# buwantaiji/FermiFlow

Hardware: AMD Instinct MI355X
Metric: walker-steps/sec (full VMC iteration: 100 MCMC steps + generate + E_loc + grad + Adam) (higher is better)
Workload: dtype f64

## Files before the change

### fermiflow_amd/csrc/ff_cnf_fwd.hip

```cpp
#include <atomic>
#include "ff_common.h"
#include "ff_ode.h"
#include "ff_slater.h"
#include "ff_eloc_ws.h"
#define FF_RADIAL_BUILD_KERNELS
#include "ff_radial.h"

#ifdef FF_STAMPS
#define FF_STAMP(i) do { unsigned long long t_ = __builtin_amdgcn_s_memtime(); stamp_acc[i] += t_ - stamp_prev; stamp_prev = t_; } while (0)
#else
#define FF_STAMP(i) do { } while (0)
#endif

#ifndef FF_TAB_MODE
#define FF_TAB_MODE(MODE) true
#endif

#include "ff_fwd_args.h"

#ifndef FF_FORM_EARLY
#define FF_FORM_EARLY 1
#endif
#ifndef FF_SWEEP_CH
#define FF_SWEEP_CH 2
#endif
#ifndef FF_FWD_WAVES_PER_SIMD
#define FF_FWD_WAVES_PER_SIMD 1
#endif
#ifndef FF_FLOW_WAVES
#define FF_FLOW_WAVES 3
#endif
#ifndef FF_FWD_STATIC
#define FF_FWD_STATIC(N, D, MODE, TAB) ((MODE) == 0 && (TAB) && (N) * (D) <= 12)
#endif
template <int N, int D, int MODE_, bool TAB>
__global__ void __launch_bounds__(FF_WAVE, ((MODE_ == 0 || MODE_ == FF_MODE_FRAMES) && TAB && N * D <= 12) ? FF_FLOW_WAVES : FF_FWD_WAVES_PER_SIMD)
ff_ode_fwd_kernel(ff_fwd_args A) {
  constexpr bool FRAMES = MODE_ == FF_MODE_FRAMES;
  constexpr int MODE = FRAMES ? 0 : MODE_;
  if constexpr (MODE == 0) FF_SETPRIO();
  using Gm = ff_geom<N, D>;
  constexpr int M = Gm::M, G = Gm::G, P = Gm::P, R = Gm::RA;
  constexpr int NH = MODE == 0 ? 1 : (MODE == 1 ? 2 : 4);
  constexpr int NV = MODE == 0 ? 1 : (MODE == 1 ? 2 : M + 5);
  constexpr int IDL = MODE == 1 ? 1 : M + 3;

  __shared__ ff_wtab s_w[TAB ? 1 : 2][TAB ? 1 : FF_HPAD];
  __shared__ double s_e2[TAB ? 1 : 64];
  __shared__ double s_z[G][M], s_kb[G][M], s_err[G][M];
  constexpr bool JET = (MODE == 2);
  constexpr bool LEAN = (MODE == 0 && TAB);
  __shared__ __attribute__((aligned(16))) double s_rr[(JET || LEAN) ? 1 : G][(JET || LEAN) ? 1 : R][2];
  __shared__ __attribute__((aligned(16))) double s_hd[JET ? 1 : G][JET ? 1 : R][NH];
  constexpr int RECW = (D + 7 + 1) & ~1;
  constexpr int RECS0 = R * RECW, RECS = RECS0 + ((RECS0 % 4 == 2) ? 0 : ((RECS0 % 4 == 0) ? 2 : 1));
  static_assert(!JET || ((2 * RECS) % 32) % 8 == 4, "record stride");
  __shared__ __attribute__((aligned(16))) double s_rec[JET ? G * RECS : 1];
  constexpr int QTW = ((3 * N > M) ? 3 * N + 1 : M + 1) | 1;
  constexpr int TROW = N * 3 * D + 1;
  static_assert(N * TROW <= M * QTW, "T must fit the transposition buffer");
  __shared__ __attribute__((aligned(16))) double s_qt[JET ? G * M * QTW : 1];
  __shared__ double s_zero[LEAN ? (D > 2 ? D : 2) : 1];
  __shared__ int s_pa[R], s_pb[R], s_any;
  __shared__ double s_rmin[G][R];
  static_assert(MODE != 2 || M <= 12, "the column-sweep local-energy kernel serves at most 12 coordinates");
  constexpr bool LDS_STATE = (MODE == 2);
  __shared__ double s_yv[LDS_STATE ? NV : 1][FF_WAVE], s_cv[LDS_STATE ? NV : 1][FF_WAVE];

  const int lane = threadIdx.x;
  const int g = lane / M, i = lane % M;
  const bool ingrp = g < G;
  const int gg = ingrp ? g : 0;
  const int ai = i / D, ci = i % D;
  const double* __restrict__ rtab = A.net.radial_table;
  if constexpr (TAB) {
    if (rtab[3] != 0.0) {
      if (lane == 0 && blockIdx.x == 0) *A.evt = A.evt_id;
      return;
    }
  } else {
    if (A.evt && *A.evt != A.evt_id) return;
    ff_fill_exp2_table(s_e2, lane);
    ff_load_weights(s_w, A.net, lane);
  }
  bool off_table = false;
  if constexpr (LEAN) { if (lane < (D > 2 ? D : 2)) s_zero[lane] = 0.0; }
  if (lane == 0) {
    int p = 0;
    for (int a = 0; a < N; a++)
      for (int b = a + 1; b < N; b++) { s_pa[p] = a; s_pb[p] = b; p++; }
    for (int a = 0; a < N; a++) { if (P + a < R) { s_pa[P + a] = a; s_pb[P + a] = -1; } }
  }
  FF_WG1_SYNC();
  const int He = A.net.He, Hm = A.net.Hm;
  const bool has_mu = Hm > 0;
  const int nrad = has_mu ? (P + N) : P;
  const double tab_inv_h = TAB ? rtab[0] : 0.0, tab_h = TAB ? rtab[1] : 0.0;
  auto heads = [&](int t, double r, double* hd) {
    if constexpr (TAB) {
      if (!ff_heads_table<NH>(rtab, tab_inv_h, tab_h, t, r, hd)) {
        off_table = true;
#pragma unroll
        for (int m = 0; m < NH; m++) hd[m] = 0.0;
      }
    } else {
      ff_heads<NH, FF_TAB_MODE(MODE)>(s_w[t], s_e2, t ? Hm : He, r, hd);
    }
  };
  const double rtol = A.rtol, atol = A.atol;
  constexpr double NT = MODE == 0 ? M : (MODE == 1 ? M + 1 : M * (M + 4) + 1);
  const int64_t ngroups = (A.B + G - 1) / G;
  __shared__ int s_st[4];
  if (lane < 4) s_st[lane] = 0;
  constexpr int NQ = (G * R + FF_WAVE - 1) / FF_WAVE;
  int rq_id[NQ];
#pragma unroll
  for (int qk = 0; qk < NQ; qk++) {
    const int q = lane + qk * FF_WAVE;
    const bool act = q < G * nrad;
    const int qg = act ? q / nrad : 0, p = act ? q - qg * nrad : 0;
    rq_id[qk] = act ? (qg | (s_pa[p] << 4) | ((s_pb[p] < 0 ? 15 : s_pb[p]) << 8) | (p << 12)) : -1;
  }
#ifdef FF_STAMPS
  unsigned long long stamp_acc[9] = {0, 0, 0, 0, 0, 0, 0, 0, 0}, stamp_prev = __builtin_amdgcn_s_memtime();
  unsigned long long stage_acc[9] = {0, 0, 0, 0, 0, 0, 0, 0, 0}, stage_cnt[9] = {0, 0, 0, 0, 0, 0, 0, 0, 0};
  const unsigned long long stamp_t0 = stamp_prev, stamp_r0 = __builtin_readcyclecounter() * 0 + wall_clock64();
#endif

  __shared__ long long s_next;
  for (int64_t grp = blockIdx.x;; grp += gridDim.x) {
    if (A.queue) {
      FF_WG1_SYNC();
      if (lane == 0) s_next = (long long)atomicAdd(A.queue + (TAB ? 0 : 1), 1ULL);
      FF_WG1_SYNC();
      grp = s_next;
    }
    if (grp >= ngroups) break;
    const int64_t bq = grp * G + g;
    const bool inb = ingrp && bq < A.B;
    const int64_t b = ff_opt_load(A.order, inb, bq, A.y_in, (int32_t)bq);
    const bool valid = inb && !(MODE == 2 && N <= 3 && A.heavy_mode == 2 && ff_opt_load(A.wclass, inb, b, A.y_in, (int32_t)0) >= A.heavy_class);
    ff_lane_vec<NV, LDS_STATE> y(&s_yv[0][0], lane), c3(&s_cv[0][0], lane);
    double c0[NV], c1[NV], c2[NV];
#pragma unroll
    for (int v = 0; v < NV; v++) { y[v] = 0.0; c0[v] = 0.0; c1[v] = 0.0; c2[v] = 0.0; c3[v] = 0.0; }
    y[0] = ff_opt_load(A.y_in, valid, b * M + i, A.y_in, 0.25 * (i + 1) + 0.125 * ((i * 7) % 5));
    if constexpr (MODE == 2) {
#pragma unroll
      for (int k = 0; k < M; k++) y[1 + k] = (k == i) ? 1.0 : 0.0;
    }
    std::conditional_t<FRAMES, ff_frame_stepper, ff_stepper> S;
    if constexpr (FRAMES) {
      S.begin(A.ta, A.tb, valid, A.nframes);
      if (valid) A.y_out[b * M + i] = y[0];
    } else {
      S.begin(A.ta, A.tb, valid);
    }
    const bool loose = MODE == 2 && ff_opt_load(A.wclass, valid, b, A.y_in, (int32_t)0x7fffffff) <= A.sens_class;
    const double hwarm = ff_open_step(ff_opt_load(A.h_init, valid, A.h_scale < 0.0 ? 0 : b, A.y_in, 0.0) * (loose ? A.h_scale_loose : fabs(A.h_scale)),
                                      A.ta, A.tb, MODE == 2 ? 0 : A.h_equal);
    const bool warm = hwarm > 0.0;
    double hmax_acc = 0.0;
    int s = -2, nev = 0;
    double h0v = 0.0, d1v = 0.0;
    double rmin_q[NQ];
#pragma unroll
    for (int k = 0; k < NQ; k++) rmin_q[k] = 1e300;

    auto group_sum = [&](double part) -> double {
      if (ingrp) s_err[g][i] = part;
      FF_WG1_SYNC();
      double t = 0.0;
#pragma unroll
      for (int j = 0; j < M; j++) t += s_err[gg][j];
      FF_WG1_SYNC();
      return t;
    };
    const double sens_w = loose ? A.sens_w : 1.0;
    auto wgt = [&](int v) -> double {
      if (MODE >= 1 && v == IDL && i != 0) return 0.0;
      return (MODE == 2 && v >= 1) ? sens_w : 1.0;
    };

    constexpr bool STATIC_STAGES = FF_FWD_STATIC(N, D, MODE, TAB);
    auto evaluate = [&](auto stage_tag) -> bool {
      constexpr int SG = decltype(stage_tag)::value;
      if constexpr (SG == FF_STAGE_DYN && STATIC_STAGES) FF_ASSUME(s <= 0);
      const int sv = SG == FF_STAGE_DYN ? s : SG;
      const double h = S.h;
      double gy = 1.0, g0 = 0.0, g1 = 0.0, g2 = 0.0;
      switch (sv) {
        case -1: g0 = h0v * S.dir; break;
        case 1: g0 = h * FF_A10; break;
        case 2: g0 = h * FF_A20; g1 = h * FF_A21; break;
        case 3: g0 = h * FF_A30; g1 = h * FF_A31; g2 = h * FF_A32; break;
        case 4: gy = 0.0; g0 = 1.0; break;
        case 5: gy = 0.0; g1 = 1.0; break;
        case 6: gy = 0.0; g2 = 1.0; break;
        default: break;
      }
      auto form = [&](double* dst, const int v0, const int v1, const int stride) {
#pragma unroll
        for (int v = v0; v < v1; v += stride) dst[v] = fma(g2, c2[v], fma(g1, c1[v], fma(g0, c0[v], gy * y[v])));
      };
      FF_STAMP(0);
      FF_WG1_SYNC();
      {
        double pub[NV];
        form(pub, 0, MODE == 2 ? M + 2 : 1, MODE == 2 ? M + 1 : 1);
        if (ingrp) {
          s_z[g][i] = pub[0];
          if constexpr (MODE == 2) s_kb[g][i] = pub[M + 1];
        }
      }
      FF_WG1_SYNC();
      FF_STAMP(1);
      double rq_rho[NQ][D], rq_dk[JET ? NQ : 1][D], rq_r[NQ], rq_ri[NQ], rq_T[NQ][TAB ? NH + 5 : 1], rq_dr[NQ];
      bool rq_ok[NQ];
#pragma unroll
      for (int qk = 0; qk < NQ; qk++) {
        const int id = rq_id[qk];
        const bool act = id >= 0;
        const int qg = act ? (id & 15) : 0, a = act ? ((id >> 4) & 15) : 0, bq = act ? ((id >> 8) & 15) : 15;
        const bool pair = bq != 15;
        const int bb = pair ? bq : a;
        double r2 = 0.0;
        const double* zpart = pair ? &s_z[qg][bb * D] : s_zero;
#pragma unroll
        for (int c = 0; c < D; c++) {
          if constexpr (LEAN) rq_rho[qk][c] = s_z[qg][a * D + c] - zpart[c];
          else rq_rho[qk][c] = s_z[qg][a * D + c] - (pair ? s_z[qg][bb * D + c] : 0.0);
          if constexpr (JET) rq_dk[qk][c] = s_kb[qg][a * D + c] - (pair ? s_kb[qg][bb * D + c] : 0.0);
          r2 = fma(rq_rho[qk][c], rq_rho[qk][c], r2);
        }
        ff_sqrt_rcp(r2, rq_r[qk], rq_ri[qk]);
        if (act) rmin_q[qk] = fmin(rmin_q[qk], rq_r[qk]);
        rq_dr[qk] = 0.0;
        rq_ok[qk] = true;
        if constexpr (TAB) {
          if constexpr (LEAN) {
            rq_ok[qk] = ff_table_fetch_always<NH>(rtab, tab_inv_h, tab_h, pair ? 0 : 1, rq_r[qk], rq_T[qk], rq_dr[qk]);
            off_table |= act & !rq_ok[qk];
          } else {
            rq_ok[qk] = ff_table_fetch<NH>(rtab, tab_inv_h, tab_h, pair ? 0 : 1, rq_r[qk], rq_T[qk], rq_dr[qk]);
            if (act && !rq_ok[qk]) off_table = true;
          }
        }
      }
      double in[NV], out[NV];
      if constexpr (MODE == 2 && FF_FORM_EARLY) form(in, 0, NV, 1);
#pragma unroll
      for (int qk = 0; qk < NQ; qk++) {
        const int id = rq_id[qk];
        if (id < 0) break;
        const int qg = id & 15, a = (id >> 4) & 15, bq = (id >> 8) & 15, p = id >> 12;
        const bool pair = bq != 15;
        const int bb = pair ? bq : a;
        const double* rho = rq_rho[qk];
        const double r = rq_r[qk], ri = rq_ri[qk];
        double hd[NH];
        if constexpr (LEAN) {
          ff_table_eval<NH>(rq_T[qk], rq_dr[qk], hd);
#pragma unroll
          for (int m = 0; m < NH; m++) hd[m] = rq_ok[qk] ? hd[m] : 0.0;
        } else if constexpr (TAB) {
          if (rq_ok[qk]) ff_table_eval<NH>(rq_T[qk], rq_dr[qk], hd);
          else {
#pragma unroll
            for (int m = 0; m < NH; m++) hd[m] = 0.0;
          }
        } else {
          heads(pair ? 0 : 1, r, hd);
        }
        if constexpr (!JET) {
          if constexpr (!LEAN) {
            s_rr[qg][p][0] = r;
            s_rr[qg][p][1] = ri;
          }
#pragma unroll
          for (int m = 0; m < NH; m++) s_hd[qg][p][m] = hd[m];
        } else {
          const double cf = pair ? 2.0 : 1.0;
          const double f0 = hd[0], f1 = hd[1], f2 = hd[NH > 2 ? 2 : 0], f3 = hd[NH > 3 ? 3 : 0];
          const double Ac = cf * fma(f2, r, (1.0 + D) * f1), Bc = cf * fma(f3, r, (2.0 + D) * f2);
          double* rec = &s_rec[qg * RECS + p * RECW];
#pragma unroll
          for (int c = 0; c < D; c++) rec[c] = rho[c];
          rec[D] = ri; rec[D + 1] = f0; rec[D + 2] = f1; rec[D + 3] = f2; rec[D + 4] = Ac; rec[D + 5] = Bc;
          rec[D + 6] = cf * fma(f1, r, D * f0);
          const double* dk = rq_dk[qk];
          double rdk = 0.0;
#pragma unroll
          for (int c = 0; c < D; c++) rdk = fma(rho[c], dk[c], rdk);
          const double F1k = f1 * (rdk * ri), gq = Ac * ri;
          double* Ta = &s_qt[qg * M * QTW + a * TROW + bb * 3 * D];
          double* Tb = &s_qt[qg * M * QTW + bb * TROW + a * 3 * D];
#pragma unroll
          for (int c = 0; c < D; c++) {
            const double pv = f0 * rho[c], pw = fma(F1k, rho[c], f0 * dk[c]), pg = gq * rho[c];
            Ta[c] = pv; Ta[D + c] = pw; Ta[2 * D + c] = pg;
            if (pair) { Tb[c] = -pv; Tb[D + c] = -pw; Tb[2 * D + c] = -pg; }
          }
        }
      }
      FF_WG1_SYNC();
      nev++;
      FF_STAMP(2);
      if constexpr (!(MODE == 2 && FF_FORM_EARLY)) form(in, 0, NV, 1);
      FF_STAMP(6);
      const double* sz = s_z[gg];
      double sumq = 0.0, ddiv = 0.0, qdiv = 0.0, divv = 0.0;
      double vi = 0.0, dvk = 0.0, gdi = 0.0;
      if constexpr (MODE == 2) {
        {
          const double* T = &s_qt[gg * M * QTW + ai * TROW + ci];
#pragma unroll
          for (int j = 0; j < N; j++) {
            const bool use = has_mu || j != ai;
            const double tv = T[j * 3 * D], tw = T[j * 3 * D + D], tg = T[j * 3 * D + 2 * D];
            vi += use ? tv : 0.0; dvk += use ? tw : 0.0; gdi += use ? tg : 0.0;
          }
        }
        FF_WG1_SYNC();
        double du[M], qv[M];
#pragma unroll
        for (int k = 0; k < M; k++) { du[k] = 0.0; qv[k] = 0.0; }
        const double* u = &in[1];
        constexpr int CH = FF_SWEEP_CH, RT = P + N, NCH = (RT + CH - 1) / CH;
        constexpr ff_pair_table<N> PT{};
        double hb[2][CH][RECW];
        auto load_chunk = [&](int c, double (*buf)[RECW]) {
#pragma unroll
          for (int q = 0; q < CH; q++) {
            const int p = c * CH + q;
            if (p < RT) {
#pragma unroll
              for (int m = 0; m < D + 7; m++) buf[q][m] = s_rec[gg * RECS + p * RECW + m];
            }
          }
        };
        load_chunk(0, hb[0]);
#pragma unroll
        for (int c = 0; c < NCH; c++) {
          if (c + 1 < NCH) load_chunk(c + 1, hb[(c + 1) & 1]);
#pragma unroll
          for (int q = 0; q < CH; q++) {
            const int p = c * CH + q;
            if (p < RT && (p < P || has_mu)) {
              const bool pair = p < P;
              const int a = pair ? PT.a[p < P ? p : 0] : p - P, bq = pair ? PT.b[p < P ? p : 0] : 0;
              const double* hq = hb[c & 1][q];
              const double* rho = hq;
              const double ri = hq[D], f0 = hq[D + 1], f1 = hq[D + 2], f2 = hq[D + 3], Ac = hq[D + 4], Bc = hq[D + 5];
              double dl[D], rd = 0.0, dd = 0.0;
#pragma unroll
              for (int cc = 0; cc < D; cc++) {
                dl[cc] = pair ? u[a * D + cc] - u[bq * D + cc] : u[a * D + cc];
                rd = fma(rho[cc], dl[cc], rd);
                dd = fma(dl[cc], dl[cc], dd);
              }
              const double r1 = rd * ri, r1s = r1 * r1;
              const double r2q = (dd - r1s) * ri;
              const double F1 = f1 * r1, F2 = fma(f2, r1s, f1 * r2q), F1x2 = F1 + F1;
#pragma unroll
              for (int cc = 0; cc < D; cc++) {
                const double g1 = fma(F1, rho[cc], f0 * dl[cc]);
                const double g2 = fma(F2, rho[cc], F1x2 * dl[cc]);
                du[a * D + cc] += g1;
                qv[a * D + cc] += g2;
                if (pair) { du[bq * D + cc] -= g1; qv[bq * D + cc] -= g2; }
              }
              ddiv = fma(Ac, r1, ddiv);
              qdiv = fma(Bc, r1s, fma(Ac, r2q, qdiv));
              divv += hq[D + 6];
            }
          }
          FF_SCHED_FENCE();
        }
        FF_STAMP(7);
#pragma unroll
        for (int k = 0; k < M; k++) out[1 + k] = du[k];
        if (ingrp) {
#pragma unroll
          for (int k = 0; k < M; k++) s_qt[(g * M + i) * QTW + k] = qv[k];
        }
        FF_WG1_SYNC();
#pragma unroll
        for (int j = 0; j < M; j++) sumq += s_qt[(gg * M + j) * QTW + i];
        FF_STAMP(3);
      } else {
        if constexpr (MODE == 1) {
          for (int p = 0; p < nrad; p++) {
            const double c = p < P ? 2.0 : 1.0;
            divv = fma(c, fma(s_hd[gg][p][NH > 1 ? 1 : 0], s_rr[gg][p][0], D * s_hd[gg][p][0]), divv);
          }
        }
        const double zc = sz[ai * D + ci];
#pragma unroll
        for (int bq = 0; bq < N; bq++) {
          const bool self = (bq == ai);
          const int lo = bq < ai ? bq : ai, hi = bq < ai ? ai : bq;
          const int p = self ? 0 : ff_pair_index(N, lo, hi);
          if constexpr (LEAN) {
            const double* hp = self ? s_zero : &s_hd[gg][p][0];
            vi = fma(*hp, zc - sz[bq * D + ci], vi);
          } else {
            vi = fma(self ? 0.0 : s_hd[gg][p][0], zc - sz[bq * D + ci], vi);
          }
        }
        if (has_mu) vi = fma(s_hd[gg][P + ai][0], zc, vi);
      }
      out[0] = vi;
      if constexpr (MODE == 1) out[1] = -divv;
      if constexpr (MODE == 2) {
        out[M + 1] = sumq + dvk;
        out[M + 2] = -ddiv;
        out[M + 3] = -divv;
        out[M + 4] = -fma(gdi, in[M + 1], qdiv);
      }
      FF_STAMP(4);
#if defined(FF_STAMPS) && defined(FF_STAMPS_TRACE)
      const int s_prev = sv;
#endif
      if (sv == -2) {
#pragma unroll
        for (int v = 0; v < NV; v++) c0[v] = out[v];
        double p0 = 0.0, p1 = 0.0;
#pragma unroll
        for (int v = 0; v < NV; v++) {
          const double isc = wgt(v) * ff_rcp(fma(fabs(y[v]), rtol, atol));
          p0 = fma(y[v] * isc, y[v] * isc, p0);
          p1 = fma(c0[v] * isc, c0[v] * isc, p1);
        }
        const double d0 = sqrt(group_sum(p0) * (1.0 / NT));
        d1v = sqrt(group_sum(p1) * (1.0 / NT));
        h0v = S.h0(d0, d1v);
        s = -1;
        if (!ff_wave_or(&s_any, lane, (!S.done && !warm) ? 1 : 0)) {
          S.habs = fmin(hwarm, S.interval);
          S.plan();
          s = 1;
        }
      } else if (sv == -1) {
        double p2 = 0.0;
#pragma unroll
        for (int v = 0; v < NV; v++) {
          const double t = (out[v] - c0[v]) * wgt(v) * ff_rcp(fma(fabs(y[v]), rtol, atol));
          p2 = fma(t, t, p2);
        }
        const double d2 = sqrt(group_sum(p2) * (1.0 / NT)) / h0v;
        S.init_habs(h0v, d1v, d2);
        if (warm) S.habs = fmin(hwarm, S.interval);
        S.plan();
        s = 1;
      } else if (sv == 0) {
#pragma unroll
        for (int v = 0; v < NV; v++) c0[v] = out[v];
        s = 1;
      } else if (sv == 1) {
#pragma unroll
        for (int v = 0; v < NV; v++) c1[v] = out[v];
        s = 2;
      } else if (sv == 2) {
#pragma unroll
        for (int v = 0; v < NV; v++) c2[v] = out[v];
        s = 3;
      } else if (sv == 3) {
#pragma unroll
        for (int v = 0; v < NV; v++) {
          const double k0v = c0[v], k1v = c1[v], k2v = c2[v], k3v = out[v];
          c0[v] = fma(h, FF_A40 * k0v + FF_A41 * k1v + FF_A42 * k2v + FF_A43 * k3v, y[v]);
          c1[v] = fma(h, FF_A50 * k0v + FF_A51 * k1v + FF_A52 * k2v + FF_A53 * k3v, y[v]);
          c2[v] = fma(h, FF_B0 * k0v + FF_B2 * k2v + FF_B3 * k3v, y[v]);
          c3[v] = h * (FF_E0 * k0v + FF_E2 * k2v + FF_E3 * k3v);
          if constexpr (STATIC_STAGES) { FF_OPAQUE(c0[v]); FF_OPAQUE(c1[v]); FF_OPAQUE(c2[v]); }
        }
        s = 4;
      } else if (sv == 4) {
#pragma unroll
        for (int v = 0; v < NV; v++) {
          c1[v] = fma(h * FF_A54, out[v], c1[v]);
          c2[v] = fma(h * FF_B4, out[v], c2[v]);
          c3[v] = fma(h * FF_E4, out[v], c3[v]);
          if constexpr (STATIC_STAGES) { FF_OPAQUE(c1[v]); FF_OPAQUE(c2[v]); }
        }
        s = 5;
      } else if (sv == 5) {
#pragma unroll
        for (int v = 0; v < NV; v++) {
          c2[v] = fma(h * FF_B5, out[v], c2[v]);
          c3[v] = fma(h * FF_E5, out[v], c3[v]);
          if constexpr (STATIC_STAGES) { FF_OPAQUE(c2[v]); }
        }
        s = 6;
      } else {
        double pe = 0.0;
#pragma unroll
        for (int v = 0; v < NV; v++) {
          const double e = fma(h * FF_E6, out[v], c3[v]);
          const double t = e * wgt(v) * ff_rcp(fma(fmax(fabs(y[v]), fabs(in[v])), rtol, atol));
          pe = fma(t, t, pe);
        }
        const double err = sqrt(group_sum(pe) * (1.0 / NT));
        const bool was_active = !S.done;
        const bool acc = S.decide(err, A.max_steps);
        if (acc) hmax_acc = fmax(hmax_acc, fabs(h));
        if (acc) {
#pragma unroll
          for (int v = 0; v < NV; v++) { y[v] = in[v]; c0[v] = out[v]; }
        }
        if constexpr (FRAMES) {
          if (valid && S.landed >= 0) A.y_out[((int64_t)S.landed * A.B + b) * M + i] = y[0];
        }
        S.plan();
        const int any = ff_wave_or(&s_any, lane, S.done ? 0 : ((was_active && !acc) ? 3 : 1));
        s = (any & 2) ? 0 : 1;
        if (!any) { FF_STAMP(5); return true; }
      }
#if defined(FF_STAMPS) && defined(FF_STAMPS_TRACE)
      { unsigned long long t_ = __builtin_amdgcn_s_memtime(); stage_acc[s_prev + 2] += t_ - stamp_prev; stage_cnt[s_prev + 2]++; }
#endif
      FF_STAMP(5);
      return false;
    };
    if constexpr (STATIC_STAGES) {
#pragma unroll 1
      for (;;) {
#pragma unroll 1
        while (s <= 0) evaluate(ff_stage_c<FF_STAGE_DYN>{});
        evaluate(ff_stage_c<1>{});
        evaluate(ff_stage_c<2>{});
        evaluate(ff_stage_c<3>{});
        evaluate(ff_stage_c<4>{});
        evaluate(ff_stage_c<5>{});
        if (evaluate(ff_stage_c<6>{})) break;
      }
    } else {
#pragma unroll 1
      for (;;) {
        if (evaluate(ff_stage_c<FF_STAGE_DYN>{})) break;
      }
    }
    if (A.wcost) {
#pragma unroll
      for (int qk = 0; qk < NQ; qk++) {
        if (rq_id[qk] >= 0) s_rmin[rq_id[qk] & 15][rq_id[qk] >> 12] = rmin_q[qk];
      }
      FF_WG1_SYNC();
    }
    if (valid) {
      const bool failed = S.fail != 0;
#ifdef FF_NO_POISON
      const double bad = 0.0;
#else
      const double bad = failed ? __builtin_nan("") : 0.0;
#endif
      if constexpr (FRAMES) {
        for (int k = S.kf; k < A.nframes; k++) A.y_out[((int64_t)k * A.B + b) * M + i] = y[0] + bad;
      } else {
        A.y_out[b * M + i] = y[0] + bad;
      }
      if constexpr (MODE >= 1) { if (i == 0) A.dl_out[b] = y[IDL] + bad; }
      if constexpr (MODE == 2) {
#pragma unroll
        for (int k = 0; k < M; k++) A.Jt[(b * M + i) * M + k] = y[1 + k];
        A.kbar[b * M + i] = y[M + 1];
        A.dD[b * M + i] = y[M + 2];
        A.Lpart[b * M + i] = y[M + 4];
      }
      if (i == 0) {
        if (A.h_out) A.h_out[b] = hmax_acc > 0.0 ? hmax_acc : hwarm;
        if (A.wcost) {
          double rm = 1e300;
          for (int p = 0; p < nrad; p++) rm = fmin(rm, s_rmin[g][p]);
          A.wcost[b] = ff_cost_class(S.nacc + S.nrej, rm);
        }
        if (A.stats) { atomicAdd(&s_st[0], nev); atomicMax(&s_st[1], S.nacc); atomicAdd(&s_st[2], S.nrej); if (failed) atomicMax(&s_st[3], 1); }
      }
    }
    FF_WG1_SYNC();
  }
#ifdef FF_STAMPS
  if (A.stats && lane == 0)
    for (int q = 0; q < 9; q++) atomicAdd((unsigned long long*)(A.stats + 8) + q, stamp_acc[q]);
  if (A.stats && lane == 0 && blockIdx.x == 0) {
    A.stats[26] = (int)(__builtin_amdgcn_s_memtime() - stamp_t0);
    A.stats[27] = (int)(wall_clock64() - stamp_r0);
  }
#ifdef FF_STAMPS_TRACE
  if (A.stats && lane == 0)
    for (int q = 0; q < 9; q++) {
      atomicAdd((unsigned long long*)(A.stats + 65600) + q, stage_acc[q]);
      atomicAdd((unsigned long long*)(A.stats + 65600) + 9 + q, stage_cnt[q]);
    }
#endif
#ifdef FF_STAMPS_TRACE
  if (A.stats && lane == 0 && blockIdx.x < 16384) {
    int* t = A.stats + 32 + 4 * blockIdx.x;
    t[0] = (int)(stamp_r0 & 0x7fffffff);
    t[1] = (int)(wall_clock64() & 0x7fffffff);
    t[2] = (int)(__builtin_amdgcn_s_memtime() - stamp_t0);
    t[3] = (int)(__builtin_amdgcn_s_getreg((4 << 0) | (0 << 6) | (31 << 11)) & 0xffff) | ((int)(__builtin_amdgcn_s_getreg((20 << 0) | (0 << 6) | (3 << 11)) & 0xf) << 16);
  }
#endif
#endif
  if constexpr (TAB) { if (off_table) *A.evt = A.evt_id; }
  FF_WG1_SYNC();
  if (A.stats && lane == 0 && (s_st[0] || s_st[3])) {
    atomicAdd(&A.stats[0], s_st[0]);
    atomicMax(&A.stats[1], s_st[1]);
    atomicAdd(&A.stats[2], s_st[2]);
    if (s_st[3]) atomicMax(&A.stats[3], 1);
  }
}


template <int N, int D, bool TAB>
__global__ void __launch_bounds__(FF_WAVE)
ff_eloc_split_kernel(ff_fwd_args A) {
  static_assert(N % 2 == 0, "split kernel needs an even particle number");
  constexpr int M = N * D, NP = N / 2, MH = NP * D, L = 2 * M, G = FF_WAVE / L;
  constexpr int P = N * (N - 1) / 2, R = P + N;
  constexpr int NV = MH + 5;
  static_assert(G >= 1, "walker does not fit a wave");

  constexpr int NH = 4;
  __shared__ ff_wtab s_w[TAB ? 1 : 2][TAB ? 1 : FF_HPAD];
  __shared__ double s_e2[TAB ? 1 : 64];
  __shared__ double s_z[G][M], s_kb[G][M], s_err[G][L];
  __shared__ double s_u[G][M][M + 1];
  constexpr int RECW = (D + 7 + 1) & ~1;
  constexpr int RECS0 = R * RECW, RECS = RECS0 + ((RECS0 % 4 == 2) ? 0 : ((RECS0 % 4 == 0) ? 2 : 1));
  __shared__ __attribute__((aligned(16))) double s_rec[G * RECS];
  constexpr int TROW = N * 3 * D + 1;
  constexpr int QTS = (N * TROW > M * 2 * (MH + 1)) ? N * TROW : M * 2 * (MH + 1);
  __shared__ double s_qt[G * QTS];
  __shared__ double s_yv[NV][FF_WAVE], s_cv[NV][FF_WAVE];
  __shared__ int s_pa[R], s_pb[R], s_any;

  const int lane = threadIdx.x;
  const int g = lane / L, idx = lane % L;
  const int h = idx / M, i = idx % M;
  const bool ingrp = g < G;
  const int gg = ingrp ? g : 0;
  const int ai = i / D, ci = i % D;
  const bool owner = (ai / NP) == h;
  const int la = owner ? ai - h * NP : -1;
  const double* __restrict__ rtab = A.net.radial_table;
  if constexpr (TAB) {
    if (rtab[3] != 0.0) {
      if (lane == 0 && blockIdx.x == 0) *A.evt = A.evt_id;
      return;
    }
  } else {
    if (A.evt && *A.evt != A.evt_id) return;
    ff_load_weights(s_w, A.net, lane);
    ff_fill_exp2_table(s_e2, lane);
  }
  bool off_table = false;
  if (lane == 0) {
    int p = 0;
    for (int a = 0; a < N; a++)
      for (int b = a + 1; b < N; b++) { s_pa[p] = a; s_pb[p] = b; p++; }
    for (int a = 0; a < N; a++) { s_pa[P + a] = a; s_pb[P + a] = -1; }
  }
  FF_WG1_SYNC();
  const int He = A.net.He, Hm = A.net.Hm;
  const bool has_mu = Hm > 0;
  const int nrad = has_mu ? R : P;
  const double tab_inv_h = TAB ? rtab[0] : 0.0, tab_h = TAB ? rtab[1] : 0.0;
  const double rtol = A.rtol, atol = A.atol;
  constexpr int NQ = (G * R + FF_WAVE - 1) / FF_WAVE;
  int rq_id[NQ];
#pragma unroll
  for (int qk = 0; qk < NQ; qk++) {
    const int q = lane + qk * FF_WAVE;
    const bool act = q < G * nrad;
    const int qg = act ? q / nrad : 0, p = act ? q - qg * nrad : 0;
    rq_id[qk] = act ? (qg | (s_pa[p] << 4) | ((s_pb[p] < 0 ? 15 : s_pb[p]) << 8) | (p << 12)) : -1;
  }
  constexpr double NT = 2.0 * M + (double)M * M + 3.0 * L;
  const int64_t ngroups = (A.B + G - 1) / G;
  __shared__ int s_st[4];
  if (lane < 4) s_st[lane] = 0;

  __shared__ long long s_next;
  for (int64_t grp = blockIdx.x;; grp += gridDim.x) {
    if (A.queue) {
      FF_WG1_SYNC();
      if (lane == 0) s_next = (long long)atomicAdd(A.queue + (TAB ? 0 : 1), 1ULL);
      FF_WG1_SYNC();
      grp = s_next;
    }
    if (grp >= ngroups) break;
    const int64_t bq = grp * G + g;
    const bool valid = ingrp && bq < A.B;
    const int64_t b = ff_opt_load(A.order, valid, bq, A.y_in, (int32_t)bq);
    ff_lane_vec<NV, true> y(&s_yv[0][0], lane), c3(&s_cv[0][0], lane);
    double c0[NV], c1[NV], c2[NV];
#pragma unroll
    for (int v = 0; v < NV; v++) { y[v] = 0.0; c0[v] = 0.0; c1[v] = 0.0; c2[v] = 0.0; c3[v] = 0.0; }
    {
      const double y0 = ff_opt_load(A.y_in, valid && owner, b * M + i, A.y_in, 0.25 * (i + 1) + 0.125 * ((i * 7) % 5));
      y[0] = owner ? y0 : y[0];
    }
#pragma unroll
    for (int k = 0; k < MH; k++) y[1 + k] = (h * MH + k == i) ? 1.0 : 0.0;
    ff_stepper S;
    S.begin(A.ta, A.tb, valid);
    const bool loose = ff_opt_load(A.wclass, valid, b, A.y_in, (int32_t)0x7fffffff) <= A.sens_class;
    const double hwarm = ff_opt_load(A.h_init, valid, A.h_scale < 0.0 ? 0 : b, A.y_in, 0.0) * (loose ? A.h_scale_loose : fabs(A.h_scale));
    const bool warm = hwarm > 0.0;
    double hmax_acc = 0.0;
    int s = -2, nev = 0;
    double h0v = 0.0, d1v = 0.0;

    auto group_sum = [&](double part) -> double {
      if (ingrp) s_err[g][idx] = part;
      FF_WG1_SYNC();
      double t = 0.0;
#pragma unroll
      for (int j = 0; j < L; j++) t += s_err[gg][j];
      FF_WG1_SYNC();
      return t;
    };
    const double sens_w = loose ? A.sens_w : 1.0;
    auto wgt = [&](int v) -> double { return ((v == 0 || v == MH + 1) && !owner) ? 0.0 : (v >= 1 ? sens_w : 1.0); };

    auto evaluate = [&](auto stage_tag) -> bool {
      constexpr int SG = decltype(stage_tag)::value;
      if constexpr (SG == FF_STAGE_DYN) FF_ASSUME(s <= 0);
      const int sv = SG == FF_STAGE_DYN ? s : SG;
      const double hs = S.h;
      double gy = 1.0, g0 = 0.0, g1 = 0.0, g2 = 0.0;
      switch (sv) {
        case -1: g0 = h0v * S.dir; break;
        case 1: g0 = hs * FF_A10; break;
        case 2: g0 = hs * FF_A20; g1 = hs * FF_A21; break;
        case 3: g0 = hs * FF_A30; g1 = hs * FF_A31; g2 = hs * FF_A32; break;
        case 4: gy = 0.0; g0 = 1.0; break;
        case 5: gy = 0.0; g1 = 1.0; break;
        case 6: gy = 0.0; g2 = 1.0; break;
        default: break;
      }
      double in[NV], out[NV];
#pragma unroll
      for (int v = 0; v < NV; v++) in[v] = fma(g2, c2[v], fma(g1, c1[v], fma(g0, c0[v], gy * y[v])));
      FF_WG1_SYNC();
      if (ingrp) {
        if (owner) { s_z[g][i] = in[0]; s_kb[g][i] = in[MH + 1]; }
#pragma unroll
        for (int k = 0; k < MH; k++) s_u[g][i][h * MH + k] = in[1 + k];
      }
      FF_WG1_SYNC();
      double rq_rho[NQ][D], rq_dk[NQ][D], rq_r[NQ], rq_ri[NQ], rq_T[NQ][TAB ? NH + 5 : 1], rq_dr[NQ];
      bool rq_ok[NQ];
#pragma unroll
      for (int qk = 0; qk < NQ; qk++) {
        const int id = rq_id[qk];
        const bool act = id >= 0;
        const int qg = act ? (id & 15) : 0, a = act ? ((id >> 4) & 15) : 0, bq = act ? ((id >> 8) & 15) : 15;
        const bool pair = bq != 15;
        const int bb = pair ? bq : a;
        double r2 = 0.0;
#pragma unroll
        for (int c = 0; c < D; c++) {
          rq_rho[qk][c] = s_z[qg][a * D + c] - (pair ? s_z[qg][bb * D + c] : 0.0);
          rq_dk[qk][c] = s_kb[qg][a * D + c] - (pair ? s_kb[qg][bb * D + c] : 0.0);
          r2 = fma(rq_rho[qk][c], rq_rho[qk][c], r2);
        }
        ff_sqrt_rcp(r2, rq_r[qk], rq_ri[qk]);
        rq_dr[qk] = 0.0;
        rq_ok[qk] = true;
        if constexpr (TAB) {
          rq_ok[qk] = ff_table_fetch<NH>(rtab, tab_inv_h, tab_h, pair ? 0 : 1, rq_r[qk], rq_T[qk], rq_dr[qk]);
          if (act && !rq_ok[qk]) off_table = true;
        }
      }
#pragma unroll
      for (int qk = 0; qk < NQ; qk++) {
        const int id = rq_id[qk];
        if (id < 0) break;
        const int qg = id & 15, a = (id >> 4) & 15, bq = (id >> 8) & 15, p = id >> 12;
        const bool pair = bq != 15;
        const int bb = pair ? bq : a;
        const double* rho = rq_rho[qk];
        const double* dk = rq_dk[qk];
        const double r = rq_r[qk], ri = rq_ri[qk];
        double hd[NH];
        if constexpr (TAB) {
          if (rq_ok[qk]) ff_table_eval<NH>(rq_T[qk], rq_dr[qk], hd);
          else {
#pragma unroll
            for (int m = 0; m < NH; m++) hd[m] = 0.0;
          }
        } else {
          ff_heads<NH, true>(s_w[pair ? 0 : 1], s_e2, pair ? He : Hm, r, hd);
        }
        const double cf = pair ? 2.0 : 1.0;
        const double f0 = hd[0], f1 = hd[1], f2 = hd[2], f3 = hd[3];
        const double Ac = cf * fma(f2, r, (1.0 + D) * f1), Bc = cf * fma(f3, r, (2.0 + D) * f2);
        double* rec = &s_rec[qg * RECS + p * RECW];
#pragma unroll
        for (int c = 0; c < D; c++) rec[c] = rho[c];
        rec[D] = ri; rec[D + 1] = f0; rec[D + 2] = f1; rec[D + 3] = f2; rec[D + 4] = Ac; rec[D + 5] = Bc;
        rec[D + 6] = cf * fma(f1, r, D * f0);
        double rdk = 0.0;
#pragma unroll
        for (int c = 0; c < D; c++) rdk = fma(rho[c], dk[c], rdk);
        const double F1k = f1 * (rdk * ri), gq = Ac * ri;
        double* Ta = &s_qt[qg * QTS + a * TROW + bb * 3 * D];
        double* Tb = &s_qt[qg * QTS + bb * TROW + a * 3 * D];
#pragma unroll
        for (int c = 0; c < D; c++) {
          const double pv = f0 * rho[c], pw = fma(F1k, rho[c], f0 * dk[c]), pg = gq * rho[c];
          Ta[c] = pv; Ta[D + c] = pw; Ta[2 * D + c] = pg;
          if (pair) { Tb[c] = -pv; Tb[D + c] = -pw; Tb[2 * D + c] = -pg; }
        }
      }
      FF_WG1_SYNC();
      nev++;
      double ddiv = 0.0, qdiv = 0.0, divv = 0.0, vi = 0.0, dvk = 0.0, gdi = 0.0;
      {
        const double* T = &s_qt[gg * QTS + ai * TROW + ci];
#pragma unroll
        for (int j = 0; j < N; j++) {
          const bool use = owner && (has_mu || j != ai);
          const double tv = T[j * 3 * D], tw = T[j * 3 * D + D], tg = T[j * 3 * D + 2 * D];
          vi += use ? tv : 0.0; dvk += use ? tw : 0.0; gdi += use ? tg : 0.0;
        }
      }
      FF_WG1_SYNC();
      double du[MH], qv[MH];
#pragma unroll
      for (int k = 0; k < MH; k++) { du[k] = 0.0; qv[k] = 0.0; }
      const double* u = &in[1];
      const double* uo = s_u[gg][i] + (1 - h) * MH;
      const int pbase = h * NP, obase = (1 - h) * NP;
      const double sg = h ? -1.0 : 1.0;
      auto term = [&](const double* rho, const double* dl, const double* rec, int m1, int m2, bool two, bool halfw) {
        double rd = 0.0, dd = 0.0;
#pragma unroll
        for (int c = 0; c < D; c++) { rd = fma(rho[c], dl[c], rd); dd = fma(dl[c], dl[c], dd); }
        const double ri = rec[D], f0 = rec[D + 1], f1 = rec[D + 2], f2 = rec[D + 3];
        const double Ac = halfw ? 0.5 * rec[D + 4] : rec[D + 4], Bc = halfw ? 0.5 * rec[D + 5] : rec[D + 5];
        const double r1 = rd * ri, r1s = r1 * r1, r2q = (dd - r1s) * ri;
        const double F1 = f1 * r1, F2 = fma(f2, r1s, f1 * r2q), F1x2 = F1 + F1;
#pragma unroll
        for (int c = 0; c < D; c++) {
          const double a1 = fma(F1, rho[c], f0 * dl[c]), a2 = fma(F2, rho[c], F1x2 * dl[c]);
          du[m1 * D + c] += a1; qv[m1 * D + c] += a2;
          if (two) { du[m2 * D + c] -= a1; qv[m2 * D + c] -= a2; }
        }
        ddiv = fma(Ac, r1, ddiv);
        qdiv = fma(Bc, r1s, fma(Ac, r2q, qdiv));
        divv = halfw ? fma(0.5, rec[D + 6], divv) : divv + rec[D + 6];
      };
#pragma unroll
      for (int m1 = 0; m1 < NP; m1++) {
#pragma unroll
        for (int m2 = m1 + 1; m2 < NP; m2++) {
          const double* rec = &s_rec[gg * RECS + ff_pair_index(N, pbase + m1, pbase + m2) * RECW];
          double dl[D];
#pragma unroll
          for (int c = 0; c < D; c++) dl[c] = u[m1 * D + c] - u[m2 * D + c];
          term(rec, dl, rec, m1, m2, true, false);
        }
        if ((m1 & 1) == 1) FF_SCHED_FENCE();
      }
#pragma unroll
      for (int m = 0; m < NP; m++) {
#pragma unroll
        for (int o = 0; o < NP; o++) {
          const int pm = pbase + m, po = obase + o;
          const double* rec = &s_rec[gg * RECS + ff_pair_index(N, pm < po ? pm : po, pm < po ? po : pm) * RECW];
          double rho[D], dl[D];
#pragma unroll
          for (int c = 0; c < D; c++) { rho[c] = sg * rec[c]; dl[c] = u[m * D + c] - uo[o * D + c]; }
          term(rho, dl, rec, m, 0, false, true);
        }
        FF_SCHED_FENCE();
      }
      if (has_mu) {
// ... 723 lines not shown
```

Measured before the change: 6.217 billion.

## Cut lean flow kernel register pressure to fit four waves per SIMD

Raises the launch-bounds occupancy target for the lean tabulated flow kernel from 3 to 4 waves per SIMD. To fit the tighter register budget, it moves per-walker open-step scalars (hwarm, h0v, d1v) into LDS and recomputes lane-derived indices (group, coordinate, walker index) at the point of use from opaque copies instead of keeping them live across the ODE loop. The aim is better latency hiding through more resident waves. The cost is extra LDS traffic and index arithmetic, and possible spills if the 4-wave budget is still too tight.

Result: faster. 6.346 billion (median of 6 runs) (+2.1%).

```diff
diff --git a/fermiflow_amd/csrc/ff_cnf_fwd.hip b/fermiflow_amd/csrc/ff_cnf_fwd.hip
--- a/fermiflow_amd/csrc/ff_cnf_fwd.hip
+++ b/fermiflow_amd/csrc/ff_cnf_fwd.hip
@@ -28,7 +28,7 @@
 #define FF_FWD_WAVES_PER_SIMD 1
 #endif
 #ifndef FF_FLOW_WAVES
-#define FF_FLOW_WAVES 3
+#define FF_FLOW_WAVES 4
 #endif
 #ifndef FF_FWD_STATIC
 #define FF_FWD_STATIC(N, D, MODE, TAB) ((MODE) == 0 && (TAB) && (N) * (D) <= 12)
@@ -66,6 +66,7 @@
   static_assert(MODE != 2 || M <= 12, "the column-sweep local-energy kernel serves at most 12 coordinates");
   constexpr bool LDS_STATE = (MODE == 2);
   __shared__ double s_yv[LDS_STATE ? NV : 1][FF_WAVE], s_cv[LDS_STATE ? NV : 1][FF_WAVE];
+  __shared__ double s_open[LEAN ? 3 : 1][LEAN ? FF_WAVE : 1];
 
   const int lane = threadIdx.x;
   const int g = lane / M, i = lane % M;
@@ -134,9 +135,14 @@
       if (lane == 0) s_next = (long long)atomicAdd(A.queue + (TAB ? 0 : 1), 1ULL);
       FF_WG1_SYNC();
       grp = s_next;
+      if constexpr (LEAN) {
+        grp = (int64_t)(((uint64_t)(uint32_t)FF_UNIFORM((int)((uint64_t)grp >> 32)) << 32) | (uint32_t)FF_UNIFORM((int)grp));
+      }
     }
     if (grp >= ngroups) break;
-    const int64_t bq = grp * G + g;
+    int lh = 0;
+    if constexpr (LEAN) { lh = lane; FF_OPAQUE(lh); }
+    const int64_t bq = grp * G + (LEAN ? lh / M : g);
     const bool inb = ingrp && bq < A.B;
     const int64_t b = ff_opt_load(A.order, inb, bq, A.y_in, (int32_t)bq);
     const bool valid = inb && !(MODE == 2 && N <= 3 && A.heavy_mode == 2 && ff_opt_load(A.wclass, inb, b, A.y_in, (int32_t)0) >= A.heavy_class);
@@ -144,6 +150,10 @@
     double c0[NV], c1[NV], c2[NV];
 #pragma unroll
     for (int v = 0; v < NV; v++) { y[v] = 0.0; c0[v] = 0.0; c1[v] = 0.0; c2[v] = 0.0; c3[v] = 0.0; }
+    if constexpr (LEAN) {
+      const int ih = lh % M;
+      y[0] = ff_opt_load(A.y_in, valid, b * M + ih, A.y_in, 0.25 * (ih + 1) + 0.125 * ((ih * 7) % 5));
+    } else
     y[0] = ff_opt_load(A.y_in, valid, b * M + i, A.y_in, 0.25 * (i + 1) + 0.125 * ((i * 7) % 5));
     if constexpr (MODE == 2) {
 #pragma unroll
@@ -152,17 +162,23 @@
     std::conditional_t<FRAMES, ff_frame_stepper, ff_stepper> S;
     if constexpr (FRAMES) {
       S.begin(A.ta, A.tb, valid, A.nframes);
-      if (valid) A.y_out[b * M + i] = y[0];
+      if (valid) A.y_out[b * M + (LEAN ? lh % M : i)] = y[0];
     } else {
       S.begin(A.ta, A.tb, valid);
     }
+    double tah = 0.0;
+    if constexpr (LEAN) { tah = A.ta; FF_OPAQUE(tah); S.interval = fabs(A.tb - tah); }
     const bool loose = MODE == 2 && ff_opt_load(A.wclass, valid, b, A.y_in, (int32_t)0x7fffffff) <= A.sens_class;
     const double hwarm = ff_open_step(ff_opt_load(A.h_init, valid, A.h_scale < 0.0 ? 0 : b, A.y_in, 0.0) * (loose ? A.h_scale_loose : fabs(A.h_scale)),
-                                      A.ta, A.tb, MODE == 2 ? 0 : A.h_equal);
+                                      LEAN ? tah : A.ta, A.tb, MODE == 2 ? 0 : A.h_equal);
     const bool warm = hwarm > 0.0;
     double hmax_acc = 0.0;
     int s = -2, nev = 0;
     double h0v = 0.0, d1v = 0.0;
+    if constexpr (LEAN) s_open[0][threadIdx.x] = hwarm;
+#define FF_OPEN_HWARM (LEAN ? s_open[0][threadIdx.x] : hwarm)
+#define FF_OPEN_H0V (LEAN ? s_open[1][threadIdx.x] : h0v)
+#define FF_OPEN_D1V (LEAN ? s_open[2][threadIdx.x] : d1v)
     double rmin_q[NQ];
 #pragma unroll
     for (int k = 0; k < NQ; k++) rmin_q[k] = 1e300;
@@ -190,7 +206,7 @@
       const double h = S.h;
       double gy = 1.0, g0 = 0.0, g1 = 0.0, g2 = 0.0;
       switch (sv) {
-        case -1: g0 = h0v * S.dir; break;
+        case -1: g0 = FF_OPEN_H0V * S.dir; break;
         case 1: g0 = h * FF_A10; break;
         case 2: g0 = h * FF_A20; g1 = h * FF_A21; break;
         case 3: g0 = h * FF_A30; g1 = h * FF_A31; g2 = h * FF_A32; break;
@@ -433,11 +449,11 @@
           p1 = fma(c0[v] * isc, c0[v] * isc, p1);
         }
         const double d0 = sqrt(group_sum(p0) * (1.0 / NT));
-        d1v = sqrt(group_sum(p1) * (1.0 / NT));
-        h0v = S.h0(d0, d1v);
+        FF_OPEN_D1V = sqrt(group_sum(p1) * (1.0 / NT));
+        FF_OPEN_H0V = S.h0(d0, FF_OPEN_D1V);
         s = -1;
         if (!ff_wave_or(&s_any, lane, (!S.done && !warm) ? 1 : 0)) {
-          S.habs = fmin(hwarm, S.interval);
+          S.habs = fmin(FF_OPEN_HWARM, S.interval);
           S.plan();
           s = 1;
         }
@@ -448,9 +464,9 @@
           const double t = (out[v] - c0[v]) * wgt(v) * ff_rcp(fma(fabs(y[v]), rtol, atol));
           p2 = fma(t, t, p2);
         }
-        const double d2 = sqrt(group_sum(p2) * (1.0 / NT)) / h0v;
-        S.init_habs(h0v, d1v, d2);
-        if (warm) S.habs = fmin(hwarm, S.interval);
+        const double d2 = sqrt(group_sum(p2) * (1.0 / NT)) / FF_OPEN_H0V;
+        S.init_habs(FF_OPEN_H0V, FF_OPEN_D1V, d2);
+        if (warm) S.habs = fmin(FF_OPEN_HWARM, S.interval);
         S.plan();
         s = 1;
       } else if (sv == 0) {
@@ -544,10 +560,23 @@
     if (A.wcost) {
 #pragma unroll
       for (int qk = 0; qk < NQ; qk++) {
+        if constexpr (LEAN) {
+          int q = lane;
+          FF_OPAQUE(q);
+          q += qk * FF_WAVE;
+          const int qg = has_mu ? q / (P + N) : q / (P > 0 ? P : 1);
+          if (q < G * nrad) s_rmin[qg][q - qg * nrad] = rmin_q[qk];
+        } else
         if (rq_id[qk] >= 0) s_rmin[rq_id[qk] & 15][rq_id[qk] >> 12] = rmin_q[qk];
       }
       FF_WG1_SYNC();
     }
+    int lt = 0;
+    int64_t bt = 0;
+    if constexpr (LEAN) { lt = lane; bt = b; FF_OPAQUE(lt); FF_OPAQUE(bt); }
+#define FF_TAIL_G (LEAN ? lt / M : g)
+#define FF_TAIL_I (LEAN ? lt % M : i)
+#define FF_TAIL_B (LEAN ? bt : b)
     if (valid) {
       const bool failed = S.fail != 0;
 #ifdef FF_NO_POISON
@@ -556,9 +585,9 @@
       const double bad = failed ? __builtin_nan("") : 0.0;
 #endif
       if constexpr (FRAMES) {
-        for (int k = S.kf; k < A.nframes; k++) A.y_out[((int64_t)k * A.B + b) * M + i] = y[0] + bad;
+        for (int k = S.kf; k < A.nframes; k++) A.y_out[((int64_t)k * A.B + FF_TAIL_B) * M + FF_TAIL_I] = y[0] + bad;
       } else {
-        A.y_out[b * M + i] = y[0] + bad;
+        A.y_out[FF_TAIL_B * M + FF_TAIL_I] = y[0] + bad;
       }
       if constexpr (MODE >= 1) { if (i == 0) A.dl_out[b] = y[IDL] + bad; }
       if constexpr (MODE == 2) {
@@ -568,17 +597,23 @@
         A.dD[b * M + i] = y[M + 2];
         A.Lpart[b * M + i] = y[M + 4];
       }
-      if (i == 0) {
-        if (A.h_out) A.h_out[b] = hmax_acc > 0.0 ? hmax_acc : hwarm;
+      if (FF_TAIL_I == 0) {
+        if (A.h_out) A.h_out[FF_TAIL_B] = hmax_acc > 0.0 ? hmax_acc : FF_OPEN_HWARM;
         if (A.wcost) {
           double rm = 1e300;
-          for (int p = 0; p < nrad; p++) rm = fmin(rm, s_rmin[g][p]);
-          A.wcost[b] = ff_cost_class(S.nacc + S.nrej, rm);
+          for (int p = 0; p < nrad; p++) rm = fmin(rm, s_rmin[FF_TAIL_G][p]);
+          A.wcost[FF_TAIL_B] = ff_cost_class(S.nacc + S.nrej, rm);
         }
         if (A.stats) { atomicAdd(&s_st[0], nev); atomicMax(&s_st[1], S.nacc); atomicAdd(&s_st[2], S.nrej); if (failed) atomicMax(&s_st[3], 1); }
       }
     }
     FF_WG1_SYNC();
+#undef FF_OPEN_HWARM
+#undef FF_OPEN_H0V
+#undef FF_OPEN_D1V
+#undef FF_TAIL_G
+#undef FF_TAIL_I
+#undef FF_TAIL_B
   }
 #ifdef FF_STAMPS
   if (A.stats && lane == 0)
```
